# sovrasov/3d-object-detection.pytorch

Hardware: AMD Instinct MI355X
Metric: regression train crops/sec @224^2 bs256 MobileNetV2 (higher is better)
Workload: dtype bf16; 1 GPU; mobilenetv2 9-class Objectron keypoint regression, train step (fwd + l1/add/CE losses + bwd + AdamW), 224x224 crops, per-GPU batch 256; global_batch=256, parallelism=dp1, roofline_sampled_steps=0, rccl_ranks=0

## Files before the change

3d-object-detection.pytorch_amd/csrc/plan.hip:

```cpp
#include <chrono>
#include <cstdio>
#include <cstdlib>
#include <cstring>
#include <string>
#include <utility>
#include <vector>

#include "common.h"

namespace {

template <class T>
inline T word_to(uint64_t v) {
  if constexpr (std::is_pointer<T>::value) {
    return reinterpret_cast<T>(static_cast<uintptr_t>(v));
  } else if constexpr (std::is_same<T, float>::value) {
    const uint32_t b = static_cast<uint32_t>(v);
    float f;
    std::memcpy(&f, &b, 4);
    return f;
  } else if constexpr (std::is_same<T, double>::value) {
    double d;
    std::memcpy(&d, &v, 8);
    return d;
// ... 4 lines not shown

template <class... A, size_t... I>
inline int call_words(int (*fn)(A...), const uint64_t* w, std::index_sequence<I...>) {
  return fn(word_to<A>(w[I])...);
}

template <class... A>
constexpr int arity(int (*)(A...)) { return (int)sizeof...(A); }

template <auto Fn>
struct Thunk;
template <class... A, int (*Fn)(A...)>
struct Thunk<Fn> {
  static int run(const uint64_t* w) { return call_words(Fn, w, std::index_sequence_for<A...>{}); }
};

struct Entry { const char* name; int (*run)(const uint64_t*); int nargs; };
#define T3D_E(fn) {#fn, &Thunk<&fn>::run, arity(&fn)}
const Entry kEntries[] = {
    T3D_E(t3d_dwconv_fwd), T3D_E(t3d_bn_finalize), T3D_E(t3d_bn_eval_affine), T3D_E(t3d_bn_eval_affine_batched),
    T3D_E(t3d_pwconv_fwd), T3D_E(t3d_pwconv_dgrad), T3D_E(t3d_pack_weight), T3D_E(t3d_sum_replicas_batched),
    T3D_E(t3d_set_dw_slots), T3D_E(t3d_set_exact_pool), T3D_E(t3d_sum_slots_batched), T3D_E(t3d_dwconv_bwd),
    T3D_E(t3d_pwconv_wgrad), T3D_E(t3d_pwconv_yfree_prep), T3D_E(t3d_pwconv_dgrad_yfree), T3D_E(t3d_pwconv_wgrad_yfree),
    T3D_E(t3d_pwconv_yfree_prep2), T3D_E(t3d_pwconv_bwd_yfree), T3D_E(t3d_pwconv_bwd_yfree_w), T3D_E(t3d_pwconv_wgrad_yfree_finish),
    T3D_E(t3d_bn_bwd_finalize), T3D_E(t3d_stem_im2col), T3D_E(t3d_stem_im2col_u8), T3D_E(t3d_crop_resize_u8),
    T3D_E(t3d_pwconv_fwd_mat), T3D_E(t3d_im2col), T3D_E(t3d_im2col_nchw), T3D_E(t3d_col2im_bwd), T3D_E(t3d_pack_conv_weight),
    T3D_E(t3d_unpack_conv_grad), T3D_E(t3d_maxpool_fwd), T3D_E(t3d_maxpool_bwd), T3D_E(t3d_res_relu_fwd),
    T3D_E(t3d_res_relu_bwd), T3D_E(t3d_subsample), T3D_E(t3d_ir_block_eval), T3D_E(t3d_bn_apply), T3D_E(t3d_bn_act_bwd),
    T3D_E(t3d_gap_fwd), T3D_E(t3d_gap_bwd), T3D_E(t3d_pool_fwd), T3D_E(t3d_pool_bwd), T3D_E(t3d_head_fwd),
    T3D_E(t3d_linear_fwd), T3D_E(t3d_head_fwd_all), T3D_E(t3d_head_bwd), T3D_E(t3d_head_bwd_weights), T3D_E(t3d_se_fwd),
    T3D_E(t3d_se_bwd), T3D_E(t3d_se_fwd_fused), T3D_E(t3d_se_bwd_data), T3D_E(t3d_se_bwd_weights), T3D_E(t3d_se_after_sums),
    T3D_E(t3d_se_after_apply), T3D_E(t3d_se_after_bwd), T3D_E(t3d_set_reduction_replicas), T3D_E(t3d_set_workspace), T3D_E(t3d_set_main_workspace),
    T3D_E(t3d_fold_request), T3D_E(t3d_pack_weights_batched), T3D_E(t3d_pwconv_pack_frag), T3D_E(t3d_adamw_step), T3D_E(t3d_set_grad_watch),
    T3D_E(t3d_sgd_step), T3D_E(t3d_rmsprop_step), T3D_E(t3d_adadelta_step),
    T3D_E(t3d_zero_batched), T3D_E(t3d_copy_cols), T3D_E(t3d_bn_bias_grad), T3D_E(t3d_se_bwd_affine), T3D_E(t3d_dropout_mask),
    T3D_E(t3d_loss_fwd_bwd), T3D_E(t3d_metrics_per_sample), T3D_E(t3d_iou3d), T3D_E(t3d_box_iou3d), T3D_E(t3d_ssd_decode_nms),
    T3D_E(t3d_expdw_fwd),
};
#undef T3D_E
constexpr int kNumEntries = (int)(sizeof(kEntries) / sizeof(kEntries[0]));
constexpr int kMaxArgs = 24;

enum OpKind { OP_CALL = 0, OP_FORK = 1, OP_COPY_D2H = 2, OP_EVENT_RECORD = 3 };
enum ArgKind { ARG_WORD = 0, ARG_STRUCT = 1, ARG_SLOT = 2 };

struct Op {
  int kind;
// ... 57 lines not shown
  if (e < 0) return T3D_ERR_UNSUPPORTED;
  if (kEntries[e].nargs != nargs) return T3D_ERR_ARG;
  Op o{};
  o.kind = OP_CALL; o.entry = e; o.nargs = nargs;
  for (int i = 0; i < nargs; ++i) {
    o.ak[i] = (uint8_t)kinds[i];
    if (kinds[i] == ARG_STRUCT) {
      const int nb = struct_bytes ? struct_bytes[i] : 0;
      if (nb <= 0 || !words[i]) return T3D_ERR_ARG;
      const size_t off = p->arena.size();
      p->arena.resize(off + (nb + 7) / 8);
      std::memcpy(&p->arena[off], reinterpret_cast<const void*>(static_cast<uintptr_t>(words[i])), nb);
      o.w[i] = off;
    } else if (kinds[i] == ARG_WORD || kinds[i] == ARG_SLOT) {
      o.w[i] = words[i];
    } else {
      return T3D_ERR_ARG;
    }
  }
  p->ops.push_back(o);
  return T3D_OK;
}

extern "C" int t3d_plan_add_fork(t3d_plan* p, void* from_stream, void* to_stream) {
  if (!p) return T3D_ERR_ARG;
  Op o{};
  o.kind = OP_FORK;
  o.w[0] = reinterpret_cast<uintptr_t>(from_stream);
  o.w[1] = reinterpret_cast<uintptr_t>(to_stream);
  if (hipEventCreateWithFlags(&o.ev, hipEventDisableTiming) != hipSuccess) return T3D_ERR_LAUNCH;
  p->ops.push_back(o);
  return T3D_OK;
}

extern "C" int t3d_plan_add_fork_after(t3d_plan* p, int producer_op, void* from_stream, void* to_stream) {
  if (!p || producer_op < 0 || producer_op >= (int)p->ops.size() || p->ops[producer_op].kind != OP_CALL) return T3D_ERR_ARG;
  Op& prod = p->ops[producer_op];
  hipStream_t from = reinterpret_cast<hipStream_t>(from_stream);
  if (prod.ev && prod.sig_stream != from) return T3D_ERR_ARG;
  if (!prod.ev) {
    if (hipEventCreateWithFlags(&prod.ev, hipEventDisableTiming) != hipSuccess) return T3D_ERR_LAUNCH;
    prod.sig_stream = from;
  }
  Op o{};
  o.kind = OP_FORK;
  o.w[0] = reinterpret_cast<uintptr_t>(from_stream);
  o.w[1] = reinterpret_cast<uintptr_t>(to_stream);
  o.w[2] = 1;
  o.ev = prod.ev;
  p->ops.push_back(o);
  return T3D_OK;
}

extern "C" int t3d_plan_add_copy_d2h(t3d_plan* p, int dst_slot, const void* src, long long bytes, void* stream) {
  if (!p || dst_slot < 0 || !src || bytes <= 0) return T3D_ERR_ARG;
  Op o{};
  o.kind = OP_COPY_D2H;
  o.w[0] = (uint64_t)dst_slot;
  o.w[1] = reinterpret_cast<uintptr_t>(src);
  o.w[2] = (uint64_t)bytes;
  o.w[3] = reinterpret_cast<uintptr_t>(stream);
  p->ops.push_back(o);
  return T3D_OK;
}
// ... 117 lines not shown
```

3d-object-detection.pytorch_amd/csrc/pwconv_common.h:

```cpp
#pragma once
#include "common.h"

namespace t3d_pw {

struct GemmArgs {
  const void* a0;
  const void* a1;
  const float *p0, *p1, *p2;
  int act, se_after, per_sample, dgrad;
  const void* w;
  const float* bias;
  const void* e_y;
  const float *e_scale, *e_shift, *e_se;
  int e_act, e_se_after;
  const void* e_res;
  void* out;
  double* stats;
  float* ps_stats;
  int ps_wave;
  int M, HW, Kin, Nout, mtiles;
  int kz;
  float* part;
  const void* a2;
  int Kin2, ks1;
  int row0;
  const T3dFold* fold;
  const void* z_res;
  void* z_out;
  int unused_[8];
  int wfrag;
  T3dQuant quant;
};

template <typename T> __device__ __forceinline__ void ldvec(const T* p, float* v);
template <> __device__ __forceinline__ void ldvec<float>(const float* p, float* v) {
  const float4 a = *reinterpret_cast<const float4*>(p);
  v[0] = a.x; v[1] = a.y; v[2] = a.z; v[3] = a.w;
}
template <> __device__ __forceinline__ void ldvec<bf16_t>(const bf16_t* p, float* v) { Vec8<bf16_t>::load(p, v); }
template <typename T> __device__ __forceinline__ void stvec(T* p, const float* v);
template <> __device__ __forceinline__ void stvec<float>(float* p, const float* v) {
  *reinterpret_cast<float4*>(p) = make_float4(v[0], v[1], v[2], v[3]);
}
template <> __device__ __forceinline__ void stvec<bf16_t>(bf16_t* p, const float* v) { Vec8<bf16_t>::store(p, v); }


int stream_launch(GemmArgs& a, hipStream_t st);
int deep_launch(GemmArgs& a, hipStream_t st);
bool deep_shape(int Kin, int Nout);
int stream_launch_f16(GemmArgs& a, hipStream_t st);
int f32_reg_launch(GemmArgs& a, hipStream_t st);

// ... 2 lines not shown
```

3d-object-detection.pytorch_amd/csrc/pwconv_stream.hip:

```cpp
#include <cstdlib>
#include <type_traits>
#include "pwconv_common.h"

#ifndef T3D_PW_F16
typedef bf16_t ST;
typedef bf16x8 ST8;
#define T3D_PW_MFMA __builtin_amdgcn_mfma_f32_16x16x32_bf16
#define T3D_PW_LAUNCH stream_launch
#else
typedef f16_t ST;
typedef f16x8 ST8;
#define T3D_PW_MFMA __builtin_amdgcn_mfma_f32_16x16x32_f16
#define T3D_PW_LAUNCH stream_launch_f16
#endif

namespace t3d_pw {
__device__ __forceinline__ f32x2 pk_fma_clamp01(f32x2 a, f32x2 b, f32x2 c) {
  f32x2 d;
  asm("v_pk_fma_f32 %0, %1, %2, %3 clamp" : "=v"(d) : "v"(a), "v"(b), "v"(c));
  return d;
}

namespace {

// ... 75 lines not shown
        const int n = n0 + (t >> 1) * 32 + ((l & 15) >> 2) * 8 + (t & 1) * 4 + (l & 3), k = ks * 32 + (l >> 4) * 8;
        ok[u] = n < a.Nout && k < a.Kin;
        v[u] = *reinterpret_cast<const ST8*>(Wg + (size_t)min(n, a.Nout - 1) * a.Kin + min(k, a.Kin - 8));
      }
#pragma unroll
      for (int u = 0; u < SU; ++u) {
        if (!ok[u]) {
#pragma unroll
          for (int j = 0; j < 8; ++j) v[u][j] = (ST)0.f;
        }
        if (i0 + u * nthr < total) Wf[i0 + u * nthr] = v[u];
      }
    }
  }
  for (int i = tid; i < BN * 2; i += nthr) { lstat[i] = 0.f; dstat[i] = 0.0; }
  for (int i = tid; i < BN; i += nthr) {
    const int n = n0 + i;
    const bool v = DG && a.e_scale && n < a.Nout;
    ecoef[i] = v ? a.e_scale[n] : 1.f;
    ecoef[BN + i] = v ? a.e_shift[n] : 0.f;
  }
  };
  constexpr bool DGL = DG && !YF;
  if (!YF && a.fold) {
    for (int i = a.Kin + tid; i < kpad; i += nthr) {
      coef[i] = DG ? 0.f : 1.f; coef[kpad + i] = 0.f; coef[2 * kpad + i] = 0.f;
    }
    t3d_fold_block(a.fold, 0, a.Kin, coef, kpad, blockIdx.x == 0, stage_weights);
  } else {
  stage_weights();
  for (int i = tid; i < kpad; i += nthr) {
    const bool v = i < a.Kin;
    if (YF) {
      coef[i] = 1.f; coef[kpad + i] = 0.f; coef[2 * kpad + i] = 0.f;
    } else if (!DG) {
      coef[i] = (v && a.p0) ? a.p0[i] : 1.f;
      coef[kpad + i] = (v && a.p0) ? a.p1[i] : 0.f;
    } else {
      coef[i] = (v && !a.per_sample) ? a.p0[i] : 0.f;
      coef[kpad + i] = v ? a.p1[i] : 0.f;
      coef[2 * kpad + i] = (v && !a.per_sample) ? a.p2[i] : 0.f;
    }
  }
  }
  __syncthreads();
  const bool c6f = !DG && !ZM && !YF && a.act == T3D_ACT_RELU6 && !(GEN && a.p2);
  if (c6f) {
// ... 207 lines not shown
                                                      min(nb + 32 * q, a.Nout - 8));
        }
        if (a.e_res) {
#pragma unroll
          for (int q = 0; q < NT / 2; ++q)
            err[q] = *reinterpret_cast<const ST8*>(reinterpret_cast<const ST*>(a.e_res) + (size_t)mld[r] * a.Nout +
                                                      min(nb + 32 * q, a.Nout - 8));
        }
      }
#pragma unroll
      for (int q = 0; q < NT / 2; ++q) {
        const int n = nb + 32 * q;
        if (n >= a.Nout) continue;
        float v[8], yv[8];
#pragma unroll
        for (int j = 0; j < 8; ++j) v[j] = acc[r][2 * q + (j >> 2)][j & 3];
        if (c6f) {
#pragma unroll
          for (int j = 0; j < 8; ++j) v[j] *= 6.f;
        }
        if ((!DG || YF) && a.bias) {
#pragma unroll
          for (int j = 0; j < 8; ++j) v[j] += a.bias[n + j];
        }
        if (DG && a.e_y) {
#pragma unroll
          for (int j = 0; j < 8; ++j) yv[j] = (float)eyr[q][j];
          if (GEN && a.e_se) {
            const float4 s0 = *reinterpret_cast<const float4*>(ecoef + (n - n0)), s1 = *reinterpret_cast<const float4*>(ecoef + (n - n0) + 4);
            const float4 h0 = *reinterpret_cast<const float4*>(ecoef + BN + (n - n0)),
                         h1 = *reinterpret_cast<const float4*>(ecoef + BN + (n - n0) + 4);
            float es[8] = {s0.x, s0.y, s0.z, s0.w, s1.x, s1.y, s1.z, s1.w};
            float eh[8] = {h0.x, h0.y, h0.z, h0.w, h1.x, h1.y, h1.z, h1.w};
            const float4 g0 = esg[GEN ? q : 0][0], g1 = esg[GEN ? q : 0][1];
            const float sv[8] = {g0.x, g0.y, g0.z, g0.w, g1.x, g1.y, g1.z, g1.w};
            if (!a.e_se_after) {
#pragma unroll
              for (int j = 0; j < 8; ++j) { es[j] *= sv[j]; eh[j] *= sv[j]; }
              act_grad_affine_vec<8>(v, yv, es, eh, a.e_act);
            } else {
              act_grad_affine_vec<8>(v, yv, es, eh, a.e_act);
#pragma unroll
              for (int j = 0; j < 8; ++j) v[j] *= sv[j];
            }
          } else if (a.e_act != T3D_ACT_NONE) {
            const float4 s0 = *reinterpret_cast<const float4*>(ecoef + (n - n0)), s1 = *reinterpret_cast<const float4*>(ecoef + (n - n0) + 4);
// ... 109 lines not shown
  const void* fn = (const void*)pw_stream_kernel<NT, R, DG, GEN, YF, KU, ZM>;
  if (lds > 64 * 1024) (void)t3d_max_lds(fn, (int)lds);
  static int occ_cache[2] = {0, 0};
  int& occ = occ_cache[threads == 512];
  if (occ == 0) {
    int n = 0;
    if (hipOccupancyMaxActiveBlocksPerMultiprocessor(&n, fn, threads, 0) != hipSuccess || n < 1) n = 1;
    occ = n;
  }
  int per_cu = occ;
  const int by_lds = (int)(160 * 1024 / (lds + 512));
  if (per_cu > by_lds) per_cu = by_lds;
  if (per_cu < 1) per_cu = 1;
  int nxb = (256 * per_cu) / nchunks;
  a.ps_wave = (ps && gps <= 16) ? 1 : 0;
  const int need = ps ? (a.ps_wave ? cdiv(a.M / a.HW, threads / 64) : a.M / a.HW) : cdiv(ngroups, threads / 64);
  if (nxb > need) nxb = need;
  if (nxb < 1) nxb = 1;
  if (nchunks > 1 && nxb >= 8) {
    const int up = (nxb + 7) & ~7;
    nxb = (up * nchunks <= 256 * per_cu) ? up : (nxb & ~7);
  }
  a.quant = (!DG && a.stats && !T3D_ENV_SET("T3D_NO_SNAP")) ? t3d_quant_for(a.M) : T3dQuant{0.0, 0.0};
  if (YF || a.per_sample) {
    if (const int rc = t3d_fold_fallback(a.p0, st)) return rc;
    a.fold = nullptr;
  } else {
    a.fold = t3d_take_fold(a.p0);
  }
  T3D_LAUNCH_TIMED((pw_stream_kernel<NT, R, DG, GEN, YF, KU, ZM>), dim3(nxb * nchunks), dim3(threads), lds, st, a, nchunks, KS,
                     g_t3d_reduce.nrep, g_t3d_reduce.stats_stride);
  T3D_CHECK_LAUNCH();
  return T3D_OK;
}

template <int NT, int R>
int launch_nt(GemmArgs& a, int KS, hipStream_t st, int deep_ku = 0) {
#ifdef T3D_PW_F16
  if (a.a2 || a.dgrad || a.z_out || a.per_sample || a.ps_stats || a.e_se || a.stats) return T3D_ERR_UNSUPPORTED;
  if (a.p2) return launch_v<NT, R, false, true>(a, KS, st);
  return launch_v<NT, R, false, false>(a, KS, st);
#else
  if (a.a2) return launch_v<NT, R, true, false, true>(a, KS, st);
  const bool gen = a.per_sample || a.ps_stats || a.e_se || (!a.dgrad && a.p2);
  if (a.dgrad && !gen && deep_ku == 3) return launch_v<NT, R, true, false, false, 3>(a, KS, st);
  if (a.dgrad && !gen && deep_ku == 5) return launch_v<NT, R, true, false, false, 5>(a, KS, st);
  if (a.dgrad) return gen ? launch_v<NT, R, true, true>(a, KS, st) : launch_v<NT, R, true, false>(a, KS, st);
// ... 57 lines not shown
```

3d-object-detection.pytorch_amd/csrc/pwconv_yfree.hip:

```cpp
#include "pwconv_common.h"

int t3d_pw_wgrad_tr_yfree(const void* dz, const void* x, float* tmp, int M, int HW, int K, int N, hipStream_t st);
size_t t3d_pw_bwd_yfree_scratch(int M, int K, int N);
int t3d_pw_bwd_yfree_launch(const void* dz, const void* x, const void* wd, const void* wt, const t3d_bnbwd* bb, const void* x_raw,
                            const void* residual, void* dx, double* stats, void* scratch, int M, int HW, int K, int N, hipStream_t st);
int t3d_pw_bwd_yfree_reduce(void* scratch, float** tmp_out, int M, int K, int N, hipStream_t st);

namespace {

__global__ __launch_bounds__(256) void yfree_prep_kernel(const bf16_t* __restrict__ wt, const float* __restrict__ alpha_g,
                                                         const float* __restrict__ beta_g, const float* __restrict__ gamma_g,
                                                         bf16_t* __restrict__ wcat, float* __restrict__ cvec, int K, int N,
                                                         int NP, int KP, const T3dFold* __restrict__ fold,
                                                         bf16_t* __restrict__ wd, int PBw) {
  extern __shared__ float fco[];
  __shared__ f32x4 red[3][64];
  const int t = threadIdx.x, lane = t & 63, wave = t >> 6, lg = lane >> 4, lc = lane & 15;
  if (fold) {
    t3d_fold_block(fold, 0, N, fco, N, blockIdx.x == 0 && blockIdx.y == 0);
  } else {
    for (int i = t; i < N; i += 256) { fco[i] = alpha_g[i]; fco[N + i] = beta_g[i]; fco[2 * N + i] = gamma_g[i]; }
    __syncthreads();
  }
  const float *alpha = fco, *beta = fco + N, *gamma = fco + 2 * N;
// ... 151 lines not shown
    return T3D_ERR_ARG;
  if (bb->per_sample) return T3D_ERR_UNSUPPORTED;
  const bool derive = true;
  const T3dFold* fold = nullptr;
  if (derive) fold = t3d_take_fold(bb->alpha);
  else if (const int rc = t3d_fold_fallback(bb->alpha, reinterpret_cast<hipStream_t>(stream))) return rc;
  T3D_LAUNCH(yfree_prep_kernel, dim3(rup32(K) / 16, rup32(K) / 16), dim3(256), (size_t)3 * N * sizeof(float),
                     reinterpret_cast<hipStream_t>(stream), reinterpret_cast<const bf16_t*>(w), bb->alpha, bb->beta, bb->gamma,
                     reinterpret_cast<bf16_t*>(wcat), cvec, K, N, rup32(N), rup32(K), fold, reinterpret_cast<bf16_t*>(wd), PBw);
  T3D_CHECK_LAUNCH();
  return T3D_OK;
}

extern "C" int t3d_pwconv_dgrad_yfree(const void* dz, const void* x, const void* wcat, const float* cvec,
                                      const void* x_raw, const t3d_prologue* pro_in, const void* residual, void* dx,
                                      double* stats, int M, int HW, int K, int N, void* stream) {
  if (!dz || !x || !wcat || !cvec || !dx || M <= 0 || HW <= 0 || K <= 0 || N <= 0 || (K % 8) || (N % 8)) return T3D_ERR_ARG;
  if (pro_in && pro_in->se) return T3D_ERR_UNSUPPORTED;
  t3d_pw::GemmArgs a{};
  a.dgrad = 1;
  a.a0 = dz; a.row0 = N;
  a.a2 = x; a.Kin2 = K; a.ks1 = rup32(N) / 32;
  a.w = wcat; a.bias = cvec; a.e_res = residual; a.out = dx; a.stats = stats;
  if (x_raw) {
    a.e_y = x_raw;
    if (pro_in) { a.e_scale = pro_in->scale; a.e_shift = pro_in->shift; a.e_act = pro_in->act; }
  }
  a.M = M; a.HW = HW; a.Kin = rup32(N) + rup32(K); a.Nout = K;
  return t3d_pw::stream_launch(a, reinterpret_cast<hipStream_t>(stream));
}

extern "C" int t3d_pwconv_wgrad_yfree(const void* dz, const void* x, const t3d_bnbwd* bb, const void* w, float* dw,
                                      int M, int HW, int K, int N, void* stream) {
  if (!dz || !x || !bb || !bb->alpha || !bb->beta || !bb->gamma || !w || !dw || M <= 0 || HW <= 0 || K <= 0 || N <= 0 ||
      (K % 8) || (N % 8))
    return T3D_ERR_ARG;
  if (bb->per_sample) return T3D_ERR_UNSUPPORTED;
  const size_t tmp_bytes = (size_t)(N + K + 8) * K * sizeof(float);
  if (!g_t3d_ws.ptr || (size_t)g_t3d_ws.bytes < 2 * tmp_bytes + (1 << 20)) return T3D_ERR_UNSUPPORTED;
  hipStream_t st = reinterpret_cast<hipStream_t>(stream);
  float* tmp = reinterpret_cast<float*>(reinterpret_cast<char*>(g_t3d_ws.ptr) + ((g_t3d_ws.bytes - tmp_bytes) & ~(size_t)255));
  const T3dWorkspace saved = g_t3d_ws;
  g_t3d_ws.bytes = reinterpret_cast<char*>(tmp) - reinterpret_cast<char*>(g_t3d_ws.ptr);
  const int rc = t3d_pw_wgrad_tr_yfree(dz, x, tmp, M, HW, K, N, st);
  g_t3d_ws = saved;
  if (rc != T3D_OK) return rc;
// ... 6 lines not shown
```

3d-object-detection.pytorch_amd/torchdet3d/_native.py:

```python
import ctypes
import os

import torch

_HERE = os.path.dirname(os.path.abspath(__file__))
LIB_PATH = os.environ.get('T3D_LIB') or os.path.join(os.path.dirname(_HERE), 'libt3d_hip.so')

W_FRAG = 0x100
F32, BF16, F16 = 0, 1, 2
ACT = {'none': 0, 'relu': 1, 'relu6': 2, 'hswish': 3}
POOL = {'avg': 0, 'max': 1, 'avg+max': 2}
_P, _I, _F, _D, _L = ctypes.c_void_p, ctypes.c_int, ctypes.c_float, ctypes.c_double, ctypes.c_longlong


class BnBwd(ctypes.Structure):
    _fields_ = [('alpha', _P), ('beta', _P), ('gamma', _P), ('per_sample', _I)]


class Prologue(ctypes.Structure):
    _fields_ = [('scale', _P), ('shift', _P), ('se', _P), ('act', _I), ('se_after_act', _I)]


class LossCfg(ctypes.Structure):
    _fields_ = [(n, _F) for n in ('c_l1', 'c_mse', 'c_smoothl1', 'smoothl1_beta', 'c_add', 'c_diag', 'c_wing',
# ... 9 lines not shown
_PP = ctypes.POINTER(Prologue)
_BP = ctypes.POINTER(BnBwd)
_LP = ctypes.POINTER(LossCfg)

SIGNATURES = {
    't3d_version': [],
    't3d_dwconv_fwd': [_I, _P, _PP, _P, _P, _P, _P, _I, _I, _I, _I, _I, _I, _P],
    't3d_bn_finalize': [_P, _I, _D, _P, _P, _P, _P, _P, _F, _F, _P, _P, _P, _P, _P],
    't3d_bn_eval_affine': [_I, _P, _P, _P, _P, _F, _P, _P, _P],
    't3d_bn_eval_affine_batched': [_P, _I, _F, _P],
    't3d_pwconv_fwd': [_I, _P, _PP, _P, _P, _P, _P, _I, _I, _I, _I, _P],
    't3d_pwconv_dgrad': [_I, _P, _P, _BP, _P, _P, _PP, _P, _P, _P, _P, _I, _I, _I, _I, _P],
    't3d_pack_weight': [_I, _P, _P, _I, _I, _I, _P],
    't3d_sum_replicas_batched': [_P, _I, _I, _P],
    't3d_set_dw_slots': [_I, _P],
    't3d_set_exact_pool': [_I],
    't3d_set_launch_events': [_P, _P],
    't3d_sum_slots_batched': [_P, _I, _P],
    't3d_dwconv_bwd': [_I, _P, _P, _BP, _P, _P, _PP, _P, _P, _P, _P, _I, _I, _I, _I, _I, _I, _P],
    't3d_pwconv_wgrad': [_I, _P, _P, _BP, _P, _PP, _P, _I, _I, _I, _I, _P],
    't3d_pwconv_yfree_prep': [_P, _BP, _P, _P, _I, _I, _P],
    't3d_pwconv_dgrad_yfree': [_P, _P, _P, _P, _P, _PP, _P, _P, _P, _I, _I, _I, _I, _P],
    't3d_pwconv_wgrad_yfree': [_P, _P, _BP, _P, _P, _I, _I, _I, _I, _P],
    't3d_pwconv_yfree_prep2': [_P, _BP, _P, _P, _P, _I, _I, _P],
    't3d_pwconv_bwd_yfree_scratch': [_I, _I, _I],
    't3d_pwconv_bwd_yfree': [_P, _P, _P, _P, _PP, _P, _P, _P, _P, _L, _I, _I, _I, _I, _P],
    't3d_pwconv_bwd_yfree_w': [_P, _P, _P, _BP, _P, _PP, _P, _P, _P, _P, _L, _I, _I, _I, _I, _P],
    't3d_pwconv_wgrad_yfree_finish': [_P, _BP, _P, _P, _I, _I, _I, _P],
    't3d_bn_bwd_finalize': [_P, _I, _D, _P, _P, _P, _P, _P, _P, _P, _P, _P],
    't3d_stem_im2col': [_I, _P, _P, _I, _I, _I, _P],
    't3d_stem_im2col_u8': [_I, _P, _P, _P, _P, _I, _I, _I, _P],
    't3d_crop_resize_u8': [_P, _P, _P, _I, _I, _I, _I, _I, _P],
    't3d_augment_crops_u8': [_P, _L, _P, _P, _I, _I, _I, _P],
    't3d_pwconv_fwd_mat': [_I, _P, _PP, _P, _P, _P, _P, _P, _I, _I, _I, _I, _P],
    't3d_ssd_decode_nms': [_I, _I, _P, _P, _P, _P, _P, _P, _P, _I, _I, _F, _F, _I, _F, _F, _P, _P, _P, _P],
    't3d_im2col': [_I, _P, _PP, _P, _I, _I, _I, _I, _I, _I, _I, _I, _P],
    't3d_im2col_nchw': [_I, _P, _P, _I, _I, _I, _I, _I, _I, _I, _I, _P],
    't3d_col2im_bwd': [_I, _P, _P, _PP, _P, _P, _I, _I, _I, _I, _I, _I, _I, _I, _P],
    't3d_pack_conv_weight': [_I, _P, _P, _I, _I, _I, _I, _P],
    't3d_unpack_conv_grad': [_P, _P, _I, _I, _I, _I, _P],
    't3d_maxpool_fwd': [_I, _P, _PP, _P, _P, _I, _I, _I, _I, _P],
    't3d_maxpool_bwd': [_I, _P, _P, _P, _PP, _P, _P, _I, _I, _I, _I, _P],
    't3d_res_relu_fwd': [_I, _P, _PP, _P, _PP, _P, _I, _I, _P],
    't3d_res_relu_bwd': [_I, _P, _P, _P, _P, _P, _P, _P, _I, _I, _P],
    't3d_subsample': [_I, _P, _P, _I, _I, _I, _I, _I, _I, _P],
    't3d_ir_block_eval': [_P, _P, _P, _P, _I, _P, _P, _P, _I, _P, _P, _P, _I, _P, _I, _I, _I, _I, _I, _I, _P],
# ... 108 lines not shown
            e.record()

    def event(self):
        return self.pool.pop() if self.pool else torch.cuda.Event(enable_timing=True)

    def per_launch(self):
        torch.cuda.synchronize()
        return [(n, sg, e0.elapsed_time(e1), nb) for (n, nb, e0, e1), sg in zip(self.rec, self.sig)]

    def summary(self):
        torch.cuda.synchronize()
        out = {}
        for name, nbytes, e0, e1 in self.rec:
            d = out.setdefault(name, dict(launches=0, ms=0.0, bytes=0))
            d['launches'] += 1
            d['ms'] += e0.elapsed_time(e1)
            d['bytes'] += nbytes or 0
        return out


timer = None
_KERNEL_TIMED = frozenset(('t3d_dwconv_fwd', 't3d_dwconv_bwd', 't3d_expdw_fwd', 't3d_pwconv_fwd', 't3d_pwconv_fwd_mat', 't3d_pwconv_dgrad',
                           't3d_pwconv_wgrad', 't3d_pwconv_dgrad_yfree', 't3d_pwconv_wgrad_yfree', 't3d_pwconv_bwd_yfree',
                           't3d_pwconv_bwd_yfree_w'))
_ABLATE = frozenset(x for x in os.environ.get('T3D_ABLATE', '').split(',') if x)


SLOT_IMGS, SLOT_GT, SLOT_CATS, SLOT_DROPOUT, SLOT_STEP, SLOT_LR, SLOT_RB_DST, SLOT_RB_EVENT, NSLOTS = range(9)
recorder = None


def call(name, *args, nbytes=None, slots=None):
    if _ABLATE and name in _ABLATE:
        return
    fn = getattr(lib(), name)
    if recorder is not None:
        recorder.add_call(name, args, nbytes, slots)
        rc = fn(*args)
        recorder.after_call()
        if rc != 0:
            raise RuntimeError(f'{name} failed with code {rc}')
        return
    t = timer
    if t is not None and (t.only is None or name in t.only):
        e0, e1 = t.event(), t.event()
        if name in _KERNEL_TIMED and t.kernel_exact:
            lib().t3d_set_launch_events(e0.cuda_event, e1.cuda_event)
# ... 136 lines not shown
```

3d-object-detection.pytorch_amd/torchdet3d/models/engine.py:

```python
import math
import os

import torch

from .. import _native as N
from .arch import Arch

BN_EPS, BN_MOM = 1e-5, 0.1
NREP = 16
FUSED_EVAL_MIN_B = int(os.environ.get('T3D_FUSED_EVAL_MIN_B', '96'))
DW_SLOTS = int(os.environ.get('T3D_DW_SLOTS', '512'))
WORKSPACE_BYTES = 64 << 20
MAIN_WORKSPACE_BYTES = 16 << 20
YFREE_MIN_ELEMS = int(os.environ.get('T3D_YFREE_MIN', 8 << 20))
YFREE_MAX_K = int(os.environ.get('T3D_YFREE_MAX_K', 112))
HOOK_MIN = 1 << 20
SE_AFTER_FUSED = None
HOOK_ON_SIDE = True


def _se_after_fused_by_shape(dt, B, HW, C, R):
    if B < 8:
        return False
    if C * R <= 4096:
# ... 332 lines not shown

    def _fold_desc(self, bn, which, count):
        key = (which, float(count))
        d = bn.desc.get(key)
        if d is None:
            f = N.BnFold()
            f.kind, f.C, f.count = which + 1, bn.C, float(count)
            f.nrep, f.rstride = bn.nrep, self._stat_stride
            f.gamma = N.ptr(bn.gamma)
            if which == 0:
                f.stats, f.beta, f.rm, f.rv, f.nbt = N.ptr(bn.stats), N.ptr(bn.beta), N.ptr(bn.rm), N.ptr(bn.rv), N.ptr(bn.nbt)
                f.momentum, f.eps = BN_MOM, BN_EPS
                f.o0, f.o1, f.o2, f.o3 = N.ptr(bn.scale), N.ptr(bn.shift), N.ptr(bn.mean), N.ptr(bn.invstd)
            else:
                f.stats, f.mean, f.invstd = N.ptr(bn.bstats), N.ptr(bn.mean), N.ptr(bn.invstd)
                f.o0, f.o1, f.o2 = N.ptr(bn.alpha), N.ptr(bn.bbeta), N.ptr(bn.gammac)
                f.o3, f.o4 = N.ptr(bn.dgamma), N.ptr(bn.dbeta)
            host = torch.frombuffer(bytearray(bytes(f)), dtype=torch.uint8)
            d = bn.desc[key] = host.to(self.device)
        return d

    _LAZY_DW = '1'
    DERIVING = frozenset(('t3d_pwconv_fwd', 't3d_pwconv_fwd_mat', 't3d_bn_apply', 't3d_pool_fwd', 't3d_pwconv_dgrad', 't3d_pwconv_yfree_prep',
                          't3d_pwconv_bwd_yfree_w', 't3d_se_bwd_affine')
                         + (('t3d_dwconv_fwd',) if _LAZY_DW in ('1', 'fwd') else ())
                         + (('t3d_dwconv_bwd',) if _LAZY_DW in ('1', 'bwd') else ()))

    def _c(self, entry, *args, fwd=None, bwd=None, **kw):
        req = False
        if fwd is not None and fwd.pend[0]:
            if self._lazy and entry in self.DERIVING:
                N.call('t3d_fold_request', N.ptr(self._fold_desc(fwd, 0, fwd.count)), N.ptr(fwd.scale))
                fwd.pend[0], req = False, True
            else:
                self._settle_f(fwd)
        if bwd is not None and bwd.pend[1]:
            if self._lazy and entry in self.DERIVING and not req:
                N.call('t3d_fold_request', N.ptr(self._fold_desc(bwd, 1, bwd.count)), N.ptr(bwd.alpha))
                bwd.pend[1], req = False, True
            else:
                self._settle_b(bwd)
        N.call(entry, *args, **kw)
        if req and N.lib().t3d_fold_pending():
            raise RuntimeError(f'{entry} left a BatchNorm finalize request unserved (engine / library mismatch)')

    def _pool_exact(self, on):
        if on != self._cur_pool_exact:
# ... 609 lines not shown

    def _hook(self, lo, on_side):
        if N.recorder is not None:
            N.recorder.host_break(('hook', lo, on_side))
        if on_side:
            with torch.cuda.stream(self._side):
                self.grad_hook(lo)
        else:
            self.grad_hook(lo)

    def _se_after_fused(self, B, HW, C, R):
        if self.arch.keys.scheme != 'timm' or C > 1024 or R > 1024:
            return False
        if SE_AFTER_FUSED is not None:
            return bool(SE_AFTER_FUSED)
        return _se_after_fused_by_shape(self.dt, B, HW, C, R)

    def _yfree_ok(self, x, M, K, Nn):
        return (self.dt == N.BF16 and YFREE_MIN_ELEMS > 0 and x.pro is None and K <= YFREE_MAX_K
                and M * Nn >= YFREE_MIN_ELEMS)

    def _expand_bwd_yfree(self, d1, bb1, bn1, wname, x, res, M, K, Nn, i):
        st = N.stream()
        tot = (Nn + 31) // 32 * 32 + (K + 31) // 32 * 32
        wcat = self._buf(f'wcat:{i}', (K, tot))
        cvec = self._buf(f'cvec:{i}', (K,), torch.float32)
        HW = x.H * x.W
        with_stats = x.bn is not None and not x.finished_act
        need = N.lib().t3d_pwconv_bwd_yfree_scratch(M, K, Nn) if not (with_stats and x.gpro is not None) else 0
        if need > 0:
            scratch = self._buf(f'yfscr:{i}', (need,), torch.uint8)
            dx = self._buf(f'dzin:{i}', (M, K))
            self._c('t3d_pwconv_bwd_yfree_w', N.ptr(d1), N.ptr(x.t), N.ptr(self.wt[wname]), bb1, N.ptr(x.raw) if with_stats else None,
                    None, N.ptr(res) if res is not None else None, N.ptr(dx), self._bst(x.bn) if with_stats else None,
                    N.ptr(scratch), need, M, HW, K, Nn, st, nbytes=M * (K + Nn) * self.esz, bwd=bn1)
            self._wgrad(N.ptr(scratch), bb1, N.ptr(self.w[wname]), N.ptr(self.g[wname]), M, K, Nn, entry='t3d_pwconv_wgrad_yfree_finish')
            if x.finished_act:
                dx = self._act_bwd(dx, x, f'dzin:{i}:a')
            return dx
        self._c('t3d_pwconv_yfree_prep', N.ptr(self.wt[wname]), bb1, N.ptr(wcat), N.ptr(cvec), K, Nn, st, bwd=bn1)
        self._wgrad(N.ptr(d1), N.ptr(x.t), bb1, N.ptr(self.w[wname]), N.ptr(self.g[wname]), M, HW, K, Nn,
                    entry='t3d_pwconv_wgrad_yfree', nbytes=M * (K + Nn) * self.esz)
        dx = self._buf(f'dzin:{i}', (M, K))
        N.call('t3d_pwconv_dgrad_yfree', N.ptr(d1), N.ptr(x.t), N.ptr(wcat), N.ptr(cvec),
               N.ptr(x.raw) if with_stats else None, x.gpro if with_stats else None,
               N.ptr(res) if res is not None else None, N.ptr(dx),
               self._bst(x.bn) if with_stats else None, M, HW, K, Nn, st, nbytes=M * (K + Nn) * self.esz)
        if x.finished_act:
            dx = self._act_bwd(dx, x, f'dzin:{i}:a')
        return dx

    def _act_bwd(self, dz, x, tag):
        M = x.B * x.H * x.W
        out = self._buf(tag, (M, x.C))
        N.call('t3d_bn_act_bwd', self.dt, N.ptr(dz), N.ptr(x.raw), x.gpro, N.ptr(out), self._bst(x.bn), M, x.C,
               N.stream())
        return out

    def _block_bwd(self, rec, dz):
        st, dt = N.stream(), self.dt
        blk, i, x, src, s2 = rec['blk'], rec['idx'], rec['x'], rec['src'], rec['s2']
        dwn, pwn = rec['names']
        B = x.B
        M2, HW2 = s2.B * s2.H * s2.W, s2.H * s2.W
        bb3 = self._bn_bwd(rec['bn3'])
        se = rec.get('se')

        def proj_wgrad():
            self._wgrad(dt, N.ptr(dz), N.ptr(rec['y3']), bb3, N.ptr(s2.t), s2.pro, N.ptr(self.g[pwn]),
                        M2, HW2, blk.cexp, blk.cout, nbytes=M2 * (blk.cexp + blk.cout) * self.esz, ro=rec['bn3'])
# ... 100 lines not shown
```

include/t3d.h:

```cpp
#ifndef T3D_H_
#define T3D_H_
#include <stdint.h>
#ifdef __cplusplus
extern "C" {
#endif

enum { T3D_F32 = 0, T3D_BF16 = 1, T3D_F16 = 2 };
enum { T3D_W_FRAG = 0x100 };
enum { T3D_ACT_NONE = 0, T3D_ACT_RELU = 1, T3D_ACT_RELU6 = 2, T3D_ACT_HSWISH = 3 };
enum { T3D_OK = 0, T3D_ERR_ARG = -1, T3D_ERR_LAUNCH = -2, T3D_ERR_UNSUPPORTED = -3 };

typedef struct {
  const float* scale;
  const float* shift;
  const float* se;
  int act;
  int se_after_act;
} t3d_prologue;

int t3d_version(void);

int t3d_dwconv_fwd(int dtype, const void* x, const t3d_prologue* pro, const float* w, void* y,
                   double* stats, float* gap_sum, int B, int H, int W, int C, int k, int stride,
                   void* stream);
// ... 19 lines not shown
                   void* y, double* stats, int M, int HW, int K, int N, void* stream);

int t3d_pwconv_frag_bytes(int rows, int cols);
int t3d_pwconv_wants_frag(int K, int N);
int t3d_pwconv_pack_frag(const void* w, void* out, int rows, int cols, void* stream);

int t3d_pwconv_dgrad(int dtype, const void* dz, const void* y, const t3d_bnbwd* bb, const void* wt,
                     const void* x_raw, const t3d_prologue* pro_in, const void* residual, void* dx,
                     double* stats, float* ps_stats, int M, int HW, int K, int N, void* stream);

int t3d_sum_replicas_batched(const long long* desc, int n, int nrep, void* stream);

int t3d_pack_weight(int dtype, const float* w, void* out, int rows, int cols, int transpose, void* stream);

int t3d_pwconv_wgrad(int dtype, const void* dz, const void* y, const t3d_bnbwd* bb, const void* x,
                     const t3d_prologue* pro, float* dw, int M, int HW, int K, int N, void* stream);

int t3d_pwconv_yfree_prep(const void* wt, const t3d_bnbwd* bb, void* wcat, float* cvec, int K, int N, void* stream);
int t3d_pwconv_dgrad_yfree(const void* dz, const void* x, const void* wcat, const float* cvec, const void* x_raw,
                           const t3d_prologue* pro_in, const void* residual, void* dx, double* stats, int M, int HW,
                           int K, int N, void* stream);
int t3d_pwconv_wgrad_yfree(const void* dz, const void* x, const t3d_bnbwd* bb, const void* w, float* dw, int M, int HW,
                           int K, int N, void* stream);

int t3d_pwconv_yfree_prep2(const void* wt, const t3d_bnbwd* bb, void* wcat, float* cvec, void* wd, int K, int N, void* stream);
int t3d_pwconv_bwd_yfree_w(const void* dz, const void* x, const void* wt, const t3d_bnbwd* bb, const void* x_raw,
                           const t3d_prologue* pro_in, const void* residual, void* dx, double* stats, void* scratch,
                           long long scratch_bytes, int M, int HW, int K, int N, void* stream);
int t3d_pwconv_bwd_yfree_scratch(int M, int K, int N);
int t3d_pwconv_bwd_yfree(const void* dz, const void* x, const void* wd, const void* x_raw, const t3d_prologue* pro_in,
                         const void* residual, void* dx, double* stats, void* scratch, long long scratch_bytes, int M, int HW,
                         int K, int N, void* stream);
int t3d_pwconv_wgrad_yfree_finish(void* scratch, const t3d_bnbwd* bb, const void* w, float* dw, int M, int K, int N, void* stream);

int t3d_dwconv_bwd(int dtype, const void* dz, const void* y, const t3d_bnbwd* bb, const float* w,
                   const void* x, const t3d_prologue* pro, const void* residual, void* dx, double* stats,
                   float* dw, int B, int H, int W, int C, int k, int stride, void* stream);

int t3d_bn_bwd_finalize(const double* stats, int C, double count, const float* gamma, const float* mean,
                        const float* invstd, float* alpha, float* beta, float* gammac, float* dgamma,
                        float* dbeta, void* stream);

int t3d_stem_im2col(int dtype, const float* x, void* col, int B, int H, int W, void* stream);
int t3d_stem_im2col_u8(int dtype, const unsigned char* x, const float* mean, const float* inv_std, void* col, int B, int H,
                       int W, void* stream);

// ... 199 lines not shown
```

Before: 38650 crops/s.

## Fuse y-free weight prep into dgrad kernel prologue, use fence-free handoff events

Adds a dgrad_yfree_w entry point. Each block builds its slice of the concatenated weight in LDS, namely alpha-scaled W plus a W·diag(beta)·Wᵀ block computed with MFMA and the gamma row sums, instead of running a separate prep kernel that writes wcat/cvec to global memory. The engine's expand-bwd path now calls this fused kernel, which removes one launch, a global round trip and a dependency. The cost is that every block recomputes the small Gram-like product redundantly. Fork events are also created with hipEventDisableSystemFence to make stream handoffs cheaper.

```diff
diff --git a/3d-object-detection.pytorch_amd/csrc/plan.hip b/3d-object-detection.pytorch_amd/csrc/plan.hip
--- a/3d-object-detection.pytorch_amd/csrc/plan.hip
+++ b/3d-object-detection.pytorch_amd/csrc/plan.hip
@@ -50,7 +50,7 @@
     T3D_E(t3d_pwconv_fwd), T3D_E(t3d_pwconv_dgrad), T3D_E(t3d_pack_weight), T3D_E(t3d_sum_replicas_batched),
     T3D_E(t3d_set_dw_slots), T3D_E(t3d_set_exact_pool), T3D_E(t3d_sum_slots_batched), T3D_E(t3d_dwconv_bwd),
     T3D_E(t3d_pwconv_wgrad), T3D_E(t3d_pwconv_yfree_prep), T3D_E(t3d_pwconv_dgrad_yfree), T3D_E(t3d_pwconv_wgrad_yfree),
-    T3D_E(t3d_pwconv_yfree_prep2), T3D_E(t3d_pwconv_bwd_yfree), T3D_E(t3d_pwconv_bwd_yfree_w), T3D_E(t3d_pwconv_wgrad_yfree_finish),
+    T3D_E(t3d_pwconv_yfree_prep2), T3D_E(t3d_pwconv_bwd_yfree), T3D_E(t3d_pwconv_bwd_yfree_w), T3D_E(t3d_pwconv_wgrad_yfree_finish), T3D_E(t3d_pwconv_dgrad_yfree_w),
     T3D_E(t3d_bn_bwd_finalize), T3D_E(t3d_stem_im2col), T3D_E(t3d_stem_im2col_u8), T3D_E(t3d_crop_resize_u8),
     T3D_E(t3d_pwconv_fwd_mat), T3D_E(t3d_im2col), T3D_E(t3d_im2col_nchw), T3D_E(t3d_col2im_bwd), T3D_E(t3d_pack_conv_weight),
     T3D_E(t3d_unpack_conv_grad), T3D_E(t3d_maxpool_fwd), T3D_E(t3d_maxpool_bwd), T3D_E(t3d_res_relu_fwd),
@@ -154,13 +154,17 @@
   return T3D_OK;
 }
 
+static hipError_t handoff_event(hipEvent_t* ev) {
+  return hipEventCreateWithFlags(ev, hipEventDisableTiming | hipEventDisableSystemFence);
+}
+
 extern "C" int t3d_plan_add_fork(t3d_plan* p, void* from_stream, void* to_stream) {
   if (!p) return T3D_ERR_ARG;
   Op o{};
   o.kind = OP_FORK;
   o.w[0] = reinterpret_cast<uintptr_t>(from_stream);
   o.w[1] = reinterpret_cast<uintptr_t>(to_stream);
-  if (hipEventCreateWithFlags(&o.ev, hipEventDisableTiming) != hipSuccess) return T3D_ERR_LAUNCH;
+  if (handoff_event(&o.ev) != hipSuccess) return T3D_ERR_LAUNCH;
   p->ops.push_back(o);
   return T3D_OK;
 }
@@ -171,7 +175,7 @@
   hipStream_t from = reinterpret_cast<hipStream_t>(from_stream);
   if (prod.ev && prod.sig_stream != from) return T3D_ERR_ARG;
   if (!prod.ev) {
-    if (hipEventCreateWithFlags(&prod.ev, hipEventDisableTiming) != hipSuccess) return T3D_ERR_LAUNCH;
+    if (handoff_event(&prod.ev) != hipSuccess) return T3D_ERR_LAUNCH;
     prod.sig_stream = from;
   }
   Op o{};
diff --git a/3d-object-detection.pytorch_amd/csrc/pwconv_common.h b/3d-object-detection.pytorch_amd/csrc/pwconv_common.h
--- a/3d-object-detection.pytorch_amd/csrc/pwconv_common.h
+++ b/3d-object-detection.pytorch_amd/csrc/pwconv_common.h
@@ -27,7 +27,8 @@
   const T3dFold* fold;
   const void* z_res;
   void* z_out;
-  int unused_[8];
+  int yfw;
+  int unused_[7];
   int wfrag;
   T3dQuant quant;
 };
diff --git a/3d-object-detection.pytorch_amd/csrc/pwconv_stream.hip b/3d-object-detection.pytorch_amd/csrc/pwconv_stream.hip
--- a/3d-object-detection.pytorch_amd/csrc/pwconv_stream.hip
+++ b/3d-object-detection.pytorch_amd/csrc/pwconv_stream.hip
@@ -121,7 +121,117 @@
   }
   };
   constexpr bool DGL = DG && !YF;
-  if (!YF && a.fold) {
+  float* const cl = coef + (YF ? a.ks1 * 32 : 0);
+  bool built = false;
+  if constexpr (YF) {
+    if (a.yfw) {
+      built = true;
+      const int K = a.Nout, Nz = a.row0, NP = a.ks1 * 32;
+      float* fco = coef;
+      auto clear = [&]() {
+        for (int i = tid; i < NT * KS * 64; i += nthr) Wf[i] = ST8{};
+        for (int i = tid; i < BN * 2; i += nthr) { lstat[i] = 0.f; dstat[i] = 0.0; }
+        for (int i = tid; i < BN; i += nthr) {
+          const int n = n0 + i;
+          const bool v = a.e_scale && n < a.Nout;
+          ecoef[i] = v ? a.e_scale[n] : 1.f;
+          ecoef[BN + i] = v ? a.e_shift[n] : 0.f;
+        }
+      };
+      if (a.fold) {
+        t3d_fold_block(a.fold, 0, Nz, fco, kpad, blockIdx.x == 0, clear);
+      } else {
+        clear();
+        for (int i = tid; i < Nz; i += nthr) { fco[i] = a.p0[i]; fco[kpad + i] = a.p1[i]; fco[2 * kpad + i] = a.p2[i]; }
+        __syncthreads();
+      }
+      const float *alpha = fco, *beta = fco + kpad, *gamma = fco + 2 * kpad;
+      ST* const Wfe = reinterpret_cast<ST*>(Wf);
+      auto fpos = [&](int nl, int col) {
+        const int t = (nl >> 5) * 2 + ((nl >> 2) & 1), l = ((col >> 3) & 3) * 16 + ((nl >> 3) & 3) * 4 + (nl & 3);
+        return ((t * KS + (col >> 5)) * 64 + l) * 8 + (col & 7);
+      };
+      const int rows = min(BN, K - n0);
+      {
+        const int nv = Nz / 8;
+        constexpr int SU = 4;
+        for (int i0 = tid; i0 < rows * nv; i0 += nthr * SU) {
+          ST8 v[SU];
+#pragma unroll
+          for (int u = 0; u < SU; ++u) {
+            const int i = min(i0 + u * nthr, rows * nv - 1);
+            v[u] = *reinterpret_cast<const ST8*>(Wg + (size_t)(n0 + i / nv) * Nz + (i % nv) * 8);
+          }
+#pragma unroll
+          for (int u = 0; u < SU; ++u) {
+            const int i = i0 + u * nthr;
+            if (i < rows * nv) {
+              const int n = (i % nv) * 8;
+              ST8 o;
+#pragma unroll
+              for (int j = 0; j < 8; ++j) o[j] = (ST)(alpha[n + j] * (float)v[u][j]);
+              *reinterpret_cast<ST8*>(Wfe + fpos(i / nv, n)) = o;
+            }
+          }
+        }
+      }
+      {
+        const int nst = (Nz + 31) / 32, nq = (K + 15) / 16, ntile = ((rows + 15) / 16) * nq;
+        for (int id = wave; id < ntile; id += WAVES) {
+          const int kt = id / nq, qt = id % nq;
+          const ST* ra = Wg + (size_t)min(n0 + kt * 16 + lc, K - 1) * Nz;
+          const ST* rb = Wg + (size_t)min(qt * 16 + lc, K - 1) * Nz;
+          f32x4 part[4];
+#pragma unroll
+          for (int w = 0; w < 4; ++w) part[w] = f32x4{0.f, 0.f, 0.f, 0.f};
+          constexpr int QU = 8;
+          for (int s0 = 0; s0 < nst; s0 += QU) {
+            ST8 fa[QU], fb[QU];
+#pragma unroll
+            for (int u = 0; u < QU; ++u) {
+              const int nc = min((s0 + u) * 32 + 8 * lg, Nz - 8);
+              fa[u] = *reinterpret_cast<const ST8*>(ra + nc);
+              fb[u] = *reinterpret_cast<const ST8*>(rb + nc);
+            }
+#pragma unroll
+            for (int u = 0; u < QU; ++u) {
+              if (s0 + u < nst) {
+                const int n = (s0 + u) * 32 + 8 * lg, nc = min(n, Nz - 8);
+                const bool live = n < Nz;
+                ST8 b;
+#pragma unroll
+                for (int j = 0; j < 8; ++j) b[j] = (ST)(live ? beta[nc + j] * (float)fb[u][j] : 0.f);
+                part[u & 3] = T3D_PW_MFMA(fa[u], b, part[u & 3], 0, 0, 0);
+              }
+            }
+          }
+          f32x4 qa = part[0];
+          qa += part[1];
+          qa += part[2];
+          qa += part[3];
+#pragma unroll
+          for (int r = 0; r < 4; ++r) {
+            const int nl = kt * 16 + 4 * lg + r, k2 = qt * 16 + lc;
+            if (nl < rows && k2 < K) Wfe[fpos(nl, NP + k2)] = (ST)qa[r];
+          }
+        }
+      }
+      for (int kb = 0; kb < BN; kb += nthr / 16) {
+        const int row = kb + (tid >> 4), sub = tid & 15;
+        float s2 = 0.f;
+        if (row < rows)
+          for (int n = sub * 8; n < Nz; n += 128) {
+            const ST8 v = *reinterpret_cast<const ST8*>(Wg + (size_t)(n0 + row) * Nz + n);
+#pragma unroll
+            for (int j = 0; j < 8; ++j) s2 = fmaf(gamma[n + j], (float)v[j], s2);
+          }
+        s2 = row16_sum(s2);
+        if (sub == 0 && row < BN) cl[row] = row < rows ? s2 : 0.f;
+      }
+    }
+  }
+  if (built) {
+  } else if (!YF && a.fold) {
     for (int i = a.Kin + tid; i < kpad; i += nthr) {
       coef[i] = DG ? 0.f : 1.f; coef[kpad + i] = 0.f; coef[2 * kpad + i] = 0.f;
     }
@@ -375,6 +485,12 @@
         if ((!DG || YF) && a.bias) {
 #pragma unroll
           for (int j = 0; j < 8; ++j) v[j] += a.bias[n + j];
+        }
+        if constexpr (YF) {
+          if (a.yfw) {
+#pragma unroll
+            for (int j = 0; j < 8; ++j) v[j] += cl[n - n0 + j];
+          }
         }
         if (DG && a.e_y) {
 #pragma unroll
@@ -530,7 +646,7 @@
     nxb = (up * nchunks <= 256 * per_cu) ? up : (nxb & ~7);
   }
   a.quant = (!DG && a.stats && !T3D_ENV_SET("T3D_NO_SNAP")) ? t3d_quant_for(a.M) : T3dQuant{0.0, 0.0};
-  if (YF || a.per_sample) {
+  if ((YF && !a.yfw) || a.per_sample) {
     if (const int rc = t3d_fold_fallback(a.p0, st)) return rc;
     a.fold = nullptr;
   } else {
diff --git a/3d-object-detection.pytorch_amd/csrc/pwconv_yfree.hip b/3d-object-detection.pytorch_amd/csrc/pwconv_yfree.hip
--- a/3d-object-detection.pytorch_amd/csrc/pwconv_yfree.hip
+++ b/3d-object-detection.pytorch_amd/csrc/pwconv_yfree.hip
@@ -197,6 +197,28 @@
   a.a0 = dz; a.row0 = N;
   a.a2 = x; a.Kin2 = K; a.ks1 = rup32(N) / 32;
   a.w = wcat; a.bias = cvec; a.e_res = residual; a.out = dx; a.stats = stats;
+  if (x_raw) {
+    a.e_y = x_raw;
+    if (pro_in) { a.e_scale = pro_in->scale; a.e_shift = pro_in->shift; a.e_act = pro_in->act; }
+  }
+  a.M = M; a.HW = HW; a.Kin = rup32(N) + rup32(K); a.Nout = K;
+  return t3d_pw::stream_launch(a, reinterpret_cast<hipStream_t>(stream));
+}
+
+extern "C" int t3d_pwconv_dgrad_yfree_w(const void* dz, const void* x, const void* wt, const t3d_bnbwd* bb, const void* x_raw,
+                                        const t3d_prologue* pro_in, const void* residual, void* dx, double* stats, int M, int HW,
+                                        int K, int N, void* stream) {
+  if (!dz || !x || !wt || !bb || !bb->alpha || !bb->beta || !bb->gamma || !dx || M <= 0 || HW <= 0 || K <= 0 || N <= 0 ||
+      (K % 8) || (N % 8))
+    return T3D_ERR_ARG;
+  if (bb->per_sample || (pro_in && pro_in->se)) return T3D_ERR_UNSUPPORTED;
+  t3d_pw::GemmArgs a{};
+  a.dgrad = 1;
+  a.yfw = 1;
+  a.a0 = dz; a.row0 = N;
+  a.a2 = x; a.Kin2 = K; a.ks1 = rup32(N) / 32;
+  a.w = wt; a.p0 = bb->alpha; a.p1 = bb->beta; a.p2 = bb->gamma;
+  a.e_res = residual; a.out = dx; a.stats = stats;
   if (x_raw) {
     a.e_y = x_raw;
     if (pro_in) { a.e_scale = pro_in->scale; a.e_shift = pro_in->shift; a.e_act = pro_in->act; }
diff --git a/3d-object-detection.pytorch_amd/torchdet3d/_native.py b/3d-object-detection.pytorch_amd/torchdet3d/_native.py
--- a/3d-object-detection.pytorch_amd/torchdet3d/_native.py
+++ b/3d-object-detection.pytorch_amd/torchdet3d/_native.py
@@ -55,6 +55,7 @@
     't3d_pwconv_yfree_prep': [_P, _BP, _P, _P, _I, _I, _P],
     't3d_pwconv_dgrad_yfree': [_P, _P, _P, _P, _P, _PP, _P, _P, _P, _I, _I, _I, _I, _P],
     't3d_pwconv_wgrad_yfree': [_P, _P, _BP, _P, _P, _I, _I, _I, _I, _P],
+    't3d_pwconv_dgrad_yfree_w': [_P, _P, _P, _BP, _P, _PP, _P, _P, _P, _I, _I, _I, _I, _P],
     't3d_pwconv_yfree_prep2': [_P, _BP, _P, _P, _P, _I, _I, _P],
     't3d_pwconv_bwd_yfree_scratch': [_I, _I, _I],
     't3d_pwconv_bwd_yfree': [_P, _P, _P, _P, _PP, _P, _P, _P, _P, _L, _I, _I, _I, _I, _P],
@@ -209,7 +210,7 @@
 timer = None
 _KERNEL_TIMED = frozenset(('t3d_dwconv_fwd', 't3d_dwconv_bwd', 't3d_expdw_fwd', 't3d_pwconv_fwd', 't3d_pwconv_fwd_mat', 't3d_pwconv_dgrad',
                            't3d_pwconv_wgrad', 't3d_pwconv_dgrad_yfree', 't3d_pwconv_wgrad_yfree', 't3d_pwconv_bwd_yfree',
-                           't3d_pwconv_bwd_yfree_w'))
+                           't3d_pwconv_bwd_yfree_w', 't3d_pwconv_dgrad_yfree_w'))
 _ABLATE = frozenset(x for x in os.environ.get('T3D_ABLATE', '').split(',') if x)
 
 
diff --git a/3d-object-detection.pytorch_amd/torchdet3d/models/engine.py b/3d-object-detection.pytorch_amd/torchdet3d/models/engine.py
--- a/3d-object-detection.pytorch_amd/torchdet3d/models/engine.py
+++ b/3d-object-detection.pytorch_amd/torchdet3d/models/engine.py
@@ -378,7 +378,7 @@
 
     _LAZY_DW = '1'
     DERIVING = frozenset(('t3d_pwconv_fwd', 't3d_pwconv_fwd_mat', 't3d_bn_apply', 't3d_pool_fwd', 't3d_pwconv_dgrad', 't3d_pwconv_yfree_prep',
-                          't3d_pwconv_bwd_yfree_w', 't3d_se_bwd_affine')
+                          't3d_pwconv_bwd_yfree_w', 't3d_pwconv_dgrad_yfree_w', 't3d_se_bwd_affine')
                          + (('t3d_dwconv_fwd',) if _LAZY_DW in ('1', 'fwd') else ())
                          + (('t3d_dwconv_bwd',) if _LAZY_DW in ('1', 'bwd') else ()))
 
@@ -1034,9 +1034,6 @@
 
     def _expand_bwd_yfree(self, d1, bb1, bn1, wname, x, res, M, K, Nn, i):
         st = N.stream()
-        tot = (Nn + 31) // 32 * 32 + (K + 31) // 32 * 32
-        wcat = self._buf(f'wcat:{i}', (K, tot))
-        cvec = self._buf(f'cvec:{i}', (K,), torch.float32)
         HW = x.H * x.W
         with_stats = x.bn is not None and not x.finished_act
         need = N.lib().t3d_pwconv_bwd_yfree_scratch(M, K, Nn) if not (with_stats and x.gpro is not None) else 0
@@ -1050,14 +1047,13 @@
             if x.finished_act:
                 dx = self._act_bwd(dx, x, f'dzin:{i}:a')
             return dx
-        self._c('t3d_pwconv_yfree_prep', N.ptr(self.wt[wname]), bb1, N.ptr(wcat), N.ptr(cvec), K, Nn, st, bwd=bn1)
+        dx = self._buf(f'dzin:{i}', (M, K))
+        self._c('t3d_pwconv_dgrad_yfree_w', N.ptr(d1), N.ptr(x.t), N.ptr(self.wt[wname]), bb1,
+                N.ptr(x.raw) if with_stats else None, x.gpro if with_stats else None,
+                N.ptr(res) if res is not None else None, N.ptr(dx),
+                self._bst(x.bn) if with_stats else None, M, HW, K, Nn, st, nbytes=M * (K + Nn) * self.esz, bwd=bn1)
         self._wgrad(N.ptr(d1), N.ptr(x.t), bb1, N.ptr(self.w[wname]), N.ptr(self.g[wname]), M, HW, K, Nn,
                     entry='t3d_pwconv_wgrad_yfree', nbytes=M * (K + Nn) * self.esz)
-        dx = self._buf(f'dzin:{i}', (M, K))
-        N.call('t3d_pwconv_dgrad_yfree', N.ptr(d1), N.ptr(x.t), N.ptr(wcat), N.ptr(cvec),
-               N.ptr(x.raw) if with_stats else None, x.gpro if with_stats else None,
-               N.ptr(res) if res is not None else None, N.ptr(dx),
-               self._bst(x.bn) if with_stats else None, M, HW, K, Nn, st, nbytes=M * (K + Nn) * self.esz)
         if x.finished_act:
             dx = self._act_bwd(dx, x, f'dzin:{i}:a')
         return dx
diff --git a/include/t3d.h b/include/t3d.h
--- a/include/t3d.h
+++ b/include/t3d.h
@@ -65,6 +65,9 @@
                            int K, int N, void* stream);
 int t3d_pwconv_wgrad_yfree(const void* dz, const void* x, const t3d_bnbwd* bb, const void* w, float* dw, int M, int HW,
                            int K, int N, void* stream);
+int t3d_pwconv_dgrad_yfree_w(const void* dz, const void* x, const void* wt, const t3d_bnbwd* bb, const void* x_raw,
+                             const t3d_prologue* pro_in, const void* residual, void* dx, double* stats, int M, int HW,
+                             int K, int N, void* stream);
 
 int t3d_pwconv_yfree_prep2(const void* wt, const t3d_bnbwd* bb, void* wcat, float* cvec, void* wd, int K, int N, void* stream);
 int t3d_pwconv_bwd_yfree_w(const void* dz, const void* x, const void* wt, const t3d_bnbwd* bb, const void* x_raw,
```

Measured after the change: 37810 crops/s. -2.2%, worse.
